# catid/siamese

Hardware: AMD Instinct MI355X
Metric: device-resident GB/s encode+decode, 1400B pkts @20% loss; % HBM peak (higher is better)
Workload: dtype u8

## Files before the change

### siamese_amd/csrc/engine.cpp

```cpp
#include "engine.h"

#include <pthread.h>
#include "backend.h"
#include "codedef.h"
#include "pool.h"

#include <algorithm>
#include <chrono>
#include <cmath>
#include <cstdio>
#include <cstddef>
#include <cstdlib>
#include <cstring>

#ifndef SGPU_EXEC_LPT
#define SGPU_EXEC_LPT 1
#endif
#ifndef SGPU_EXEC_GROUPS
#define SGPU_EXEC_GROUPS 256
#endif

namespace sgpu {

void EngineStats::add(const EngineStats& o)
// ... 28 lines not shown
namespace {

uint64_t now_ns()
{
    return (uint64_t)std::chrono::duration_cast<std::chrono::nanoseconds>(
               std::chrono::steady_clock::now().time_since_epoch())
        .count();
}

inline size_t align16(size_t v) { return (v + 15) & ~(size_t)15; }

}


namespace {
std::mutex g_bodyMu;
std::vector<ProgramBody*> g_bodies;
}

ProgramBody* ProgramBody::get()
{
    {
        std::lock_guard<std::mutex> g(g_bodyMu);
        if (!g_bodies.empty()) {
            ProgramBody* b = g_bodies.back();
            g_bodies.pop_back();
            return b;
        }
    }
    return new ProgramBody;
}

void ProgramBody::put(ProgramBody* b)
{
    b->clear();
    std::lock_guard<std::mutex> g(g_bodyMu);
    if (g_bodies.size() < (1u << 15))
        g_bodies.push_back(b);
    else
        delete b;
}

void ProgramBody::clear()
{
    for (size_t k = 0; k < nsegs; ++k)
        segs[k].clear();
    nsegs = 0;
    resultWords = 0;
    nsolves = 0;
    nges = 0;
    callbacks.clear();
    keep.clear();
    rb.open = false;
    rb.win.clear();
    rb.updates.clear();
    rb.rows.clear();
    copies.clear();
    lcb.clear();
    ndeliver = 0;
    nframe = 0;
    frameLit.clear();
    frameLitRefs.clear();
    nrelay = 0;
    npackjob = npack = 0;
    nconcatjob = nconcat = 0;
    gateOpen = false;
}

void ProgramBody::new_segment()
{
    rows_close();
    if (nsegs == segs.size())
        segs.emplace_back();
    segs[nsegs++].clear();
}

void ProgramBody::rows_open(uint32_t base, bool keepWindow)
{
    rows_close();
    if (nsegs == 0)
        new_segment();
    rb.open = true;
    rb.haveSums = false;
    rb.sumsVersion = 0;
    rb.readMask = 0;
    rb.cutMax = 0;
    rb.versioned = false;
    if (!keepWindow) {
        rb.base = base;
        rb.win.clear();
    }
    rb.updates.clear();
    for (int& u : rb.updateOf)
        u = -1;
    rb.rows.clear();
    rb.maxExtent = 0;
}

namespace {
inline bool overlaps(uint64_t a, uint64_t an, uint64_t b, uint64_t bn) { return a < b + bn && b < a + an; }
inline uint64_t lane_span(uint32_t n) { return ((uint64_t)n + 15) & ~(uint64_t)15; }
}

void ProgramBody::lc_seal()
{
    if (lcb.items.empty())
        return;
    Segment& s = segs[nsegs - 1];
    if (lcb.items.size() == 1) {
        const LcItem& it = lcb.items[0];
        GfOp op;
        std::memset(&op, 0, sizeof(op));
        op.dst = it.dst;
        op.n = it.n;
        op.valid = it.valid;
        op.kind = OP_LINCOMB;
        op.mix = it.mixLit & 0xff;
        op.termBegin = (uint32_t)s.terms.size();
        op.termCount = it.termCount;
        s.ops.push_back(op);
        s.terms.insert(s.terms.end(), lcb.terms.begin(), lcb.terms.end());
        const uint32_t litLen = (it.mixLit >> 8) & 0xff;
        if (litLen) {
            GfOp lo;
            std::memset(&lo, 0, sizeof(lo));
            lo.dst = it.dst;
            lo.n = it.litOffset;
            lo.valid = litLen;
            lo.kind = OP_LITERAL;
            std::memcpy(lo.lit, it.lit, litLen);
            s.ops.push_back(lo);
        }
        lcb.clear();
        return;
    }
    const uint32_t itemWords = (uint32_t)lcb.items.size() * kLcWords;
    for (LcItem& it : lcb.items)
        it.termStart += itemWords;
    GfOp op;
    std::memset(&op, 0, sizeof(op));
    op.kind = OP_LINCOMBS;
    op.n = (uint32_t)lcb.items.size();
    op.termBegin = (uint32_t)(s.rowsData.size() / 16);
    op.termCount = itemWords + (uint32_t)lcb.terms.size();
    s.ops.push_back(op);
    const size_t at = s.rowsData.size();
    s.rowsData.resize(at + (size_t)op.termCount * 16);
    std::memcpy(s.rowsData.data() + at, lcb.items.data(), lcb.items.size() * sizeof(LcItem));
    std::memcpy(s.rowsData.data() + at + lcb.items.size() * sizeof(LcItem), lcb.terms.data(),
                lcb.terms.size() * sizeof(GfTerm));
    s.rowsWords += op.termCount;
    lcb.clear();
}

namespace {

using Span = ProgramBody::LcBuild::Span;

bool span_hits(const std::vector<Span>& v, uint64_t lo, uint64_t hi)
{
    const auto it = std::upper_bound(v.begin(), v.end(), lo,
                                     [](uint64_t x, const Span& sp) { return x < sp.hi; });
    return it != v.end() && it->lo < hi;
}

void span_add(std::vector<Span>& v, uint64_t lo, uint64_t hi)
{
    if (lo >= hi)
        return;
    auto first = std::lower_bound(v.begin(), v.end(), lo,
                                  [](const Span& sp, uint64_t x) { return sp.hi < x; });
    auto last = first;
    while (last != v.end() && last->lo <= hi) {
        lo = std::min(lo, last->lo);
        hi = std::max(hi, last->hi);
        ++last;
    }
    if (first == last) {
        v.insert(first, Span{lo, hi});
    } else {
        *first = Span{lo, hi};
        v.erase(first + 1, last);
    }
}

uint64_t lc_write_span(const LcItem& it)
{
    const uint32_t litEnd = it.litOffset + ((it.mixLit >> 8) & 0xff);
    return std::max<uint64_t>(lane_span(it.n), litEnd);
}

}

void ProgramBody::lc_absorb()
{
    static const bool enabled = [] {
        const char* v = std::getenv("SIAMESE_AMD_LC_BATCH");
        return !v || std::atoi(v) != 0;
    }();
    if (!enabled)
        return;
    Segment& s = segs[nsegs - 1];
    const GfOp op = s.ops.back();
// ... 6 lines not shown
    }
    bool indep = lcb.items.size() < kLcMaxItems;
    const uint64_t w = lane_span(op.n);
    if (indep && !lcb.items.empty()) {
        if (span_hits(lcb.writes, op.dst, op.dst + w) || span_hits(lcb.reads, op.dst, op.dst + w))
            indep = false;
        for (uint32_t k = 0; indep && k < op.termCount; ++k)
            if (span_hits(lcb.writes, t[k].src, t[k].src + lane_span(t[k].len)))
                indep = false;
        const LcItem& it = lcb.items.back();
        const uint64_t iw = lc_write_span(it);
        if (indep && overlaps(op.dst, w, it.dst, iw))
            indep = false;
        for (uint32_t k = 0; indep && k < op.termCount; ++k)
            if (overlaps(t[k].src, lane_span(t[k].len), it.dst, iw))
                indep = false;
        const GfTerm* u = lcb.terms.data() + it.termStart;
        for (uint32_t k = 0; indep && k < it.termCount; ++k)
            if (overlaps(u[k].src, lane_span(u[k].len), op.dst, w))
                indep = false;
    }
    lcScratch.assign(t, t + op.termCount);
    s.terms.resize(op.termBegin);
    s.ops.pop_back();
    if (!indep) {
        lc_seal();
    } else if (!lcb.items.empty()) {
        const LcItem& it = lcb.items.back();
        span_add(lcb.writes, it.dst, it.dst + lc_write_span(it));
        const GfTerm* u = lcb.terms.data() + it.termStart;
        for (uint32_t k = 0; k < it.termCount; ++k)
            span_add(lcb.reads, u[k].src, u[k].src + lane_span(u[k].len));
    }
    LcItem it;
    std::memset(&it, 0, sizeof(it));
    it.dst = op.dst;
    it.n = op.n;
    it.valid = op.valid;
    it.termStart = (uint32_t)lcb.terms.size();
    it.termCount = op.termCount;
    it.mixLit = op.mix & 0xff;
    lcb.items.push_back(it);
    lcb.terms.insert(lcb.terms.end(), lcScratch.begin(), lcScratch.end());
}

bool ProgramBody::lc_literal_fits(uint64_t at, uint32_t len) const
{
    return !span_hits(lcb.writes, at, at + len) && !span_hits(lcb.reads, at, at + len);
}

void ProgramBody::rows_close()
{
    lc_seal();
    if (!copies.empty()) {
        Segment& g = segs[nsegs - 1];
        GfOp op;
        std::memset(&op, 0, sizeof(op));
        op.kind = OP_COPIES;
        op.n = (uint32_t)copies.size();
        op.termBegin = (uint32_t)(g.rowsData.size() / 16);
        op.termCount = (uint32_t)copies.size() * kCopyWords;
        g.ops.push_back(op);
        const size_t at = g.rowsData.size();
        g.rowsData.resize(at + copies.size() * sizeof(CopyItem));
        std::memcpy(g.rowsData.data() + at, copies.data(), copies.size() * sizeof(CopyItem));
        g.rowsWords += op.termCount;
        copies.clear();
    }
    RowsBuild& b = rb;
    if (!b.open)
        return;
    b.open = false;
    if (b.rows.empty() && b.updates.empty())
        return;
    if (!b.haveSums)
        std::memset(b.sums, 0, sizeof(b.sums));
    Segment& s = segs[nsegs - 1];
    const size_t winKept = b.win.size();
    for (RowItem& r : b.rows) {
        if (r.ldpcN < kLdpcSplitMin)
            continue;
        const uint32_t entry = (uint32_t)b.win.size();
        const uint32_t pairs = (r.ldpcN + kPairRate - 1) / kPairRate;
        s.wide.push_back(Segment::Wide{(uint32_t)s.ops.size(), entry, r.n, r.row, r.ldpcN, r.ldpcOff});
        s.wideItems += ((r.n + kLdpcTileBytes - 1) / kLdpcTileBytes) *
                       ((pairs + ldpc_pairs_per_item(r.n) - 1) / ldpc_pairs_per_item(r.n));
        s.wideBytes += 2 * (uint64_t)((r.n + kLdpcTileBytes - 1) / kLdpcTileBytes * kLdpcTileBytes);
        WinEntry z;
        std::memset(&z, 0, sizeof(z));
        b.win.push_back(z);
        b.win.push_back(z);
        r.ldpcN = 0;
        r.ldpcOff = entry;
        r.mask0 |= kRowWide;
    }
    const uint32_t E = (uint32_t)b.win.size();
    const uint32_t U = (uint32_t)b.updates.size();
    const uint32_t R = (uint32_t)b.rows.size();
    const uint32_t words = kRowSums + E + U * kUpdateWords + R * kRowWords;
    uint32_t stageLo = E;
    for (const SumUpdate& u : b.updates)
        if (u.to > u.from)
            stageLo = std::min(stageLo, u.from);
    for (const RowItem& r : b.rows)
        if (r.ldpcN || (r.mask0 & kRowWide))
            stageLo = std::min(stageLo, r.ldpcOff);
    GfOp op;
    std::memset(&op, 0, sizeof(op));
    op.dst = stageLo | (uint64_t)(b.versioned ? std::min<uint32_t>(R, kVersionRows) : 0u) << 32;
    op.kind = OP_ROWS;
    op.n = R;
    op.valid = E;
    op.mix = U;
    op.termBegin = (uint32_t)(s.rowsData.size() / 16);
    op.termCount = words;
    s.ops.push_back(op);
    const size_t at = s.rowsData.size();
    s.rowsData.resize(at + (size_t)words * 16);
    uint8_t* w = s.rowsData.data() + at;
    std::memcpy(w, b.sums, sizeof(b.sums));
    w += sizeof(b.sums);
    std::memcpy(w, b.win.data(), (size_t)E * sizeof(WinEntry));
    w += (size_t)E * sizeof(WinEntry);
    std::memcpy(w, b.updates.data(), (size_t)U * sizeof(SumUpdate));
    w += (size_t)U * sizeof(SumUpdate);
    std::memcpy(w, b.rows.data(), (size_t)R * sizeof(RowItem));
    b.win.resize(winKept);
    s.rowsWords += words;
    if (b.maxExtent > s.maxExtent)
        s.maxExtent = b.maxExtent;
}


Program::~Program()
{
    if (!shard_) {
        if (b_)
            ProgramBody::put(b_);
        return;
    }
    Program* orphan = new Program(eng_, group_ | 2);
    orphan->shard_ = shard_;
    orphan->b_ = b_;
    b_ = nullptr;
    std::lock_guard<std::mutex> g(shard_->mu);
    auto it = std::find(shard_->dirty.begin(), shard_->dirty.end(), this);
    if (it != shard_->dirty.end())
        *it = orphan;
}

void Program::attach()
{
    if (!b_)
        b_ = ProgramBody::get();
    b_->group = group_ & 1;
    Shard& s = eng_->shard();
    shard_ = &s;
    std::lock_guard<std::mutex> g(s.mu);
    s.dirty.push_back(this);
}

void Program::lc_begin(uint64_t dst, uint32_t n, uint32_t valid, uint8_t mix)
{
    touch();
    if (b_->rb.open || !b_->copies.empty()) {
        b_->lc_seal();
        b_->rows_close();
    }
    if (b_->nsegs == 0)
        b_->new_segment();
    ProgramBody::Segment& s = b_->segs[b_->nsegs - 1];
    GfOp op;
    op.dst = dst;
    op.n = n;
    op.valid = valid < n ? valid : n;
    op.kind = OP_LINCOMB;
    op.mix = mix;
    op.termBegin = (uint32_t)s.terms.size();
    op.termCount = 0;
    s.ops.push_back(op);
}

void Program::lc_end()
{
    ProgramBody::Segment& s = b_->segs[b_->nsegs - 1];
    GfOp& op = s.ops.back();
    if (op.termCount == 0 && op.valid >= op.n) {
        s.ops.pop_back();
        return;
    }
    if (op.n > s.maxExtent)
        s.maxExtent = op.n;
    b_->lc_absorb();
}

void Program::add_mem(uint64_t dst, uint64_t src, uint32_t n)
{
    if (n == 0)
        return;
    lc_begin(dst, n, n);
    lc_term(src, n, 1);
    lc_end();
}

void Program::muladd_mem(uint64_t dst, uint8_t y, uint64_t src, uint32_t n)
{
    if (n == 0 || y == 0)
        return;
    lc_begin(dst, n, n);
    lc_term(src, n, y);
    lc_end();
}

void Program::mul_mem(uint64_t dst, uint64_t src, uint8_t y, uint32_t n)
{
    if (n == 0)
        return;
    lc_begin(dst, n, 0);
// ... 50 lines not shown

void Program::ingest_device(const DevBuf& dst, uint64_t src, uint32_t bytes, const uint8_t* hdr,
                            uint32_t hdrLen)
{
    ingest_run(dst.addr(), 0, src, 0, 1, bytes, hdr, hdrLen);
}

void Program::ingest_run(uint64_t dst, uint32_t dstStride, uint64_t src, uint32_t srcStride, uint32_t count,
                         uint32_t bytes, const uint8_t* hdr, uint32_t hdrLen)
{
    IngestDesc d;
    std::memset(&d, 0, sizeof(d));
    d.dst = dst;
    d.src = src;
    d.bytes = bytes;
    d.hdrLen = hdrLen;
    d.count = count;
    d.srcStride = count > 1 ? srcStride : 0;
    d.dstStride = count > 1 ? dstStride : 0;
    std::memcpy(d.hdr, hdr, hdrLen < 8 ? hdrLen : 8);
    eng_->add_ingest(d, -1);
}

uint32_t Program::solve(const std::vector<SolveRow>& rows, const uint8_t* coef, uint32_t maxBytes)
{
    SolveRow* r = nullptr;
    uint8_t* c = nullptr;
    solve_reserve((unsigned)rows.size(), &r, &c);
    std::memcpy(r, rows.data(), rows.size() * sizeof(SolveRow));
    std::memcpy(c, coef, rows.size() * rows.size());
    return solve_commit(maxBytes);
}

void Program::solve_reserve(unsigned m, SolveRow** rows, uint8_t** coef)
{
    touch();
    if (b_->nsegs == 0)
        b_->new_segment();
    if (b_->nsolves == b_->solves.size())
        b_->solves.emplace_back();
    ProgramBody::PendingSolve& ps = b_->solves[b_->nsolves];
    ps.rows.resize(m);
    ps.coef.resize((size_t)m * m);
    *rows = ps.rows.data();
    *coef = ps.coef.data();
}

uint32_t Program::solve_commit(uint32_t maxBytes, uint32_t gateWord)
{
    ProgramBody::PendingSolve& ps = b_->solves[b_->nsolves++];
    const size_t m = ps.rows.size();
    DevBuf head = eng_->alloc((uint32_t)m * 16u);
    if (head) {
        if (b_->copies.empty()) {
            b_->rows_close();
            if (b_->nsegs == 0)
                b_->new_segment();
        }
        std::vector<CopyItem>& cp = b_->copies;
        size_t at = cp.size();
        cp.resize(at + m);
        uint32_t ext = 0;
        for (size_t i = 0; i < m; ++i) {
            const uint32_t len = std::min<uint32_t>(16u, ps.rows[i].initBytes);
            if (len == 0)
                continue;
            CopyItem& c = cp[at++];
            std::memset(&c, 0, sizeof(c));
            c.dst = head.addr() + i * 16;
            c.src = ps.rows[i].buf;
            c.len = len;
            ext = std::max(ext, len);
        }
        cp.resize(at);
        ProgramBody::Segment& g = b_->segs[b_->nsegs - 1];
        if (ext > g.maxExtent)
            g.maxExtent = ext;
        b_->rows_close();
    }
    std::memset(&ps.desc, 0, sizeof(ps.desc));
    ps.desc.head = head.addr();
    eng_->release(head);
    ps.desc.m = (uint32_t)m;
    ps.desc.maxBytes = maxBytes;
    ps.desc.gate = gateWord;
    if (gateWord && b_->nges) {
        ProgramBody::PendingGe& g = b_->ges[b_->nges - 1];
        g.solve = (uint32_t)(b_->nsolves - 1);
    }
    ps.desc.result = b_->resultWords;
    b_->resultWords += ps.desc.m + 2;
    const uint32_t r = ps.desc.result;
    b_->new_segment();
    return r;
}

void Program::gate_begin(uint32_t word)
{
    touch();
    b_->rows_close();
    if (b_->nsegs == 0)
        b_->new_segment();
    b_->gateOpen = true;
    b_->gateSeg = b_->nsegs - 1;
    b_->gateOp = (uint32_t)b_->segs[b_->nsegs - 1].ops.size();
    b_->gateWord = word;
}

uint32_t Program::gate_end()
{
    if (!b_ || !b_->gateOpen)
        return 0;
    b_->rows_close();
    b_->gateOpen = false;
    ProgramBody::Segment& s = b_->segs[b_->gateSeg];
    uint32_t wide = 0;
    if (b_->gateSeg + 1 == b_->nsegs && s.ops.size() > b_->gateOp) {
        s.gates.push_back(ProgramBody::Segment::Gate{b_->gateOp, (uint32_t)s.ops.size(), b_->gateWord});
        for (const ProgramBody::Segment::Wide& x : s.wide)
            wide += x.op >= b_->gateOp;
    }
    return wide;
}

uint8_t* Program::ge_job(unsigned rows, unsigned cols, unsigned pickLen, uint32_t* resultWord, bool chained)
{
    touch();
    if (b_->nges == b_->ges.size())
        b_->ges.emplace_back();
    ProgramBody::PendingGe& g = b_->ges[b_->nges++];
    g.rows = (uint16_t)rows;
    g.cols = (uint16_t)cols;
    g.pickLen = pickLen;
    g.result = b_->resultWords;
    g.chained = chained;
    g.solve = ~0u;
    b_->resultWords += ge_result_words(rows, cols, chained);
    g.in.resize(ge_input_bytes(rows, cols, pickLen));
    *resultWord = g.result;
    return g.in.data();
}

void Program::on_complete(Completion fn)
{
    touch();
    b_->callbacks.push_back(std::move(fn));
}

void Program::on_complete(std::shared_ptr<void> keep, Completion fn)
{
    touch();
    b_->keep.push_back(std::move(keep));
    b_->callbacks.push_back(std::move(fn));
}


WinEntry* Program::rows_window(uint32_t lo, uint32_t hi, uint32_t* from)
{
    touch();
    ProgramBody::RowsBuild& b = b_->rb;
    if (!b.open || lo < b.base)
        rows_open(lo, false);
    const uint32_t end = b.base + (uint32_t)b.win.size();
    if (hi <= end) {
        *from = hi;
        return nullptr;
    }
    *from = end;
    b.win.resize(hi - b.base);
    return b.win.data() + (end - b.base);
}

void Program::rows_update(unsigned k, uint64_t dst, uint32_t n, uint32_t valid, unsigned s,
                          uint32_t fromElement, uint32_t toElement)
{
    ProgramBody::RowsBuild& b = b_->rb;
    if (b.readMask >> k & 1) {
        const WinEntry& seen = b.sums[k];
        if (seen.src != dst || valid < seen.len || toElement - fromElement > kVersionMaxSpan ||
            b.rows.size() >= kVersionRows)
            rows_open(b.base, true);
        else
            b.versioned = true;
    }
    const uint32_t from = fromElement - b.base, to = toElement - b.base;
    int& ui = b.updateOf[k];
    if (ui >= 0) {
        SumUpdate& u = b.updates[ui];
        const uint64_t d = ((uint64_t)u.dstHi << 32) | u.dstLo;
        if (d == dst && (u.to == from || from == to)) {
            if (from != to)
                u.to = to;
            if (n > u.n)
                u.n = n;
            if (n > b.maxExtent)
                b.maxExtent = n;
            return;
        }
        rows_open(b.base, true);
    }
    SumUpdate u;
    std::memset(&u, 0, sizeof(u));
    u.dstLo = (uint32_t)dst;
    u.dstHi = (uint32_t)(dst >> 32);
    u.n = n;
    u.valid = valid < n ? valid : n;
    u.s = s;
    u.from = from;
    u.to = to < from ? from : to;
    u.sum = k;
    b.updateOf[k] = (int)b.updates.size();
    b.updates.push_back(u);
    if (n > b.maxExtent)
        b.maxExtent = n;
}

uint64_t Program::next_table_version()
{
    static std::atomic<uint64_t> next{1};
    return next.fetch_add(1, std::memory_order_relaxed);
}

void Program::rows_row(const WinEntry* sums, uint64_t dst, uint32_t n, uint32_t valid, uint8_t mix,
                       uint32_t mask0, uint32_t mask1, unsigned row, uint32_t ldpcN,
                       uint32_t ldpcFirst, uint32_t cutoff, const uint8_t* lit, uint32_t litLen,
                       uint64_t sumsVersion)
{
    ProgramBody::RowsBuild& b = b_->rb;
    const bool unchanged = sumsVersion != 0 && b.haveSums && b.sumsVersion == sumsVersion;
    bool same = true;
    if (b.haveSums && !unchanged)
        for (uint32_t r = b.readMask; r; r &= r - 1) {
            const unsigned k = (unsigned)__builtin_ctz(r);
            if (std::memcmp(&b.sums[k], &sums[k], sizeof(WinEntry)) != 0) {
                same = false;
                break;
            }
        }
    if (!same || cutoff < b.cutMax || (b.versioned && b.rows.size() >= kVersionRows))
        rows_open(b.base, true);
    b.cutMax = std::max(b.cutMax, cutoff);
    if (!(unchanged && b.haveSums))
        std::memcpy(b.sums, sums, sizeof(b.sums));
    b.haveSums = true;
    b.sumsVersion = sumsVersion;
    RowItem r;
    std::memset(&r, 0, sizeof(r));
    r.dst = dst;
    r.n = n;
    r.valid = valid < n ? valid : n;
    r.mask0 = mask0 | (litLen << 24);
    r.mask1 = mask1 | ((uint32_t)mix << 24);
    r.row = row;
    r.ldpcN = ldpcN;
    r.ldpcOff = ldpcFirst - b.base;
    r.cutoff = cutoff - b.base;
    if (litLen)
        std::memcpy(r.lit, lit, litLen);
    b.rows.push_back(r);
    b.readMask |= mask0 | mask1;
    if (n + litLen > b.maxExtent)
        b.maxExtent = n + litLen;
}

void Program::copy(uint64_t dst, uint64_t src, uint32_t len)
{
    if (len == 0)
        return;
    touch();
    if (b_->copies.empty()) {
        b_->rows_close();
        if (b_->nsegs == 0)
            b_->new_segment();
    }
    CopyItem c;
    std::memset(&c, 0, sizeof(c));
    c.dst = dst;
    c.src = src;
    c.len = len;
    b_->copies.push_back(c);
    ProgramBody::Segment& g = b_->segs[b_->nsegs - 1];
    if (len > g.maxExtent)
        g.maxExtent = len;
}

void Program::deliver(uint64_t src, uint32_t cap, uint64_t dst, uint64_t lenOut, uint64_t stride)
{
    touch();
    DeliverItem it;
    it.src = src;
    it.dst = dst;
    it.lenOut = lenOut;
    it.cap = cap;
    it.stride16 = (uint32_t)(stride >> 4);
    if (b_->ndeliver == b_->delivers.size())
        b_->delivers.emplace_back();
    b_->delivers[b_->ndeliver++] = it;
}

void Program::frame(uint64_t src, uint32_t bytes, const uint8_t* hdr, uint32_t hdrLen, uint64_t dst,
                    uint64_t lenOut, uint64_t stride, uint32_t lenBase)
{
    touch();
    FrameItem it;
    it.src = src;
    it.dst = dst;
    it.lenOut = lenOut;
    it.bytes = bytes;
    it.stride16 = (uint32_t)(stride >> 4);
    std::memset(it.hdr, 0, sizeof(it.hdr));
    std::memcpy(it.hdr, hdr, hdrLen);
    it.hdrLen = (uint8_t)hdrLen;
    it.lenBase = lenBase;
    if (b_->nframe == b_->frames.size())
        b_->frames.emplace_back();
    b_->frames[b_->nframe++] = it;
}

void Program::frame_literal(const uint8_t* data, uint32_t bytes, const uint8_t* hdr, uint32_t hdrLen, uint64_t dst,
                            uint64_t lenOut, uint64_t stride)
{
    touch();
    const size_t at = b_->frameLit.size();
    b_->frameLit.resize(align16(at + bytes), 0);
    std::memcpy(b_->frameLit.data() + at, data, bytes);
    b_->frameLitRefs.push_back(ProgramBody::FrameLitRef{b_->nframe, (uint32_t)at});
    frame(1 , bytes, hdr, hdrLen, dst, lenOut, stride);
}

void Program::relay(uint64_t src, uint32_t cap, uint32_t flow, uint32_t packetNum, uint64_t dst, uint64_t lenOut,
                    uint64_t stride)
{
    touch();
    RelayItem it;
// ... 615 lines not shown
constexpr size_t kAcctBytes = 32;

constexpr size_t kParallelWords = 1u << 16;
#ifndef SGPU_SEAL_CHUNK
#define SGPU_SEAL_CHUNK 32
#endif
#ifndef SGPU_SEG_CHUNK
#define SGPU_SEG_CHUNK 16
#endif
#ifndef SGPU_INGEST_CHUNK
#define SGPU_INGEST_CHUNK 8192
#endif
#ifndef SGPU_SOLVE_CHUNK
#define SGPU_SOLVE_CHUNK 64
#endif

std::atomic<bool> g_measureUnique{false};

struct Range
{
    uint64_t addr;
    uint32_t len;
};

uint64_t distinct_bytes(std::vector<Range>& v)
{
    std::sort(v.begin(), v.end(), [](const Range& a, const Range& b) { return a.addr < b.addr; });
    uint64_t total = 0;
    for (size_t i = 0; i < v.size();) {
        uint32_t len = v[i].len;
        size_t j = i + 1;
        for (; j < v.size() && v[j].addr == v[i].addr; ++j)
            len = std::max(len, v[j].len);
        total += len;
        i = j;
    }
    return total;
}

uint64_t segment_unique_bytes(const ProgramBody::Segment& s, std::vector<Range>& rd, std::vector<Range>& wr)
{
    rd.clear();
    wr.clear();
    uint64_t words = 0;
    auto R = [&](uint64_t a, uint32_t n) {
        if (a && n)
            rd.push_back(Range{a, n});
    };
    auto W = [&](uint64_t a, uint32_t n, uint32_t valid) {
        if (a && n)
            wr.push_back(Range{a, n});
        R(a, std::min(valid, n));
    };
    for (const GfOp& op : s.ops) {
        words += op_words(op);
        const uint8_t* blk = s.rowsData.data() + (size_t)op.termBegin * 16;
        switch (op.kind) {
        case OP_LINCOMB:
            W(op.dst, op.n, op.valid);
            for (uint32_t t = 0; t < op.termCount; ++t)
                R(s.terms[op.termBegin + t].src, s.terms[op.termBegin + t].len);
            break;
        case OP_LITERAL:
            W(op.dst + op.n, op.valid, 0);
            break;
        case OP_ROWS: {
            const WinEntry* sums = reinterpret_cast<const WinEntry*>(blk);
            const WinEntry* win = sums + kRowSums;
            const SumUpdate* up = reinterpret_cast<const SumUpdate*>(win + op.valid);
            const RowItem* rows = reinterpret_cast<const RowItem*>(up + op.mix);
            for (unsigned k = 0; k < kRowSums; ++k)
                R(sums[k].src, sums[k].len);
            for (uint32_t e = (uint32_t)op.dst; e < op.valid; ++e)
                R(win[e].src, win[e].len);
            for (uint32_t u = 0; u < op.mix; ++u)
                W((uint64_t)up[u].dstHi << 32 | up[u].dstLo, up[u].n, up[u].valid);
            for (uint32_t r = 0; r < op.n; ++r)
                W(rows[r].dst, rows[r].n + row_lit_len(rows[r].mask0), rows[r].valid);
            break;
        }
        case OP_COPIES: {
            const CopyItem* c = reinterpret_cast<const CopyItem*>(blk);
            for (uint32_t i = 0; i < op.n; ++i) {
                W(c[i].dst, c[i].len, 0);
                R(c[i].src, c[i].len);
            }
            break;
        }
        case OP_LINCOMBS: {
            const LcItem* it = reinterpret_cast<const LcItem*>(blk);
            for (uint32_t i = 0; i < op.n; ++i) {
                W(it[i].dst, std::max(it[i].n, it[i].litOffset + ((it[i].mixLit >> 8) & 0xff)), it[i].valid);
                const GfTerm* t = reinterpret_cast<const GfTerm*>(blk + (size_t)it[i].termStart * 16);
                for (uint32_t k = 0; k < it[i].termCount; ++k)
                    R(t[k].src, t[k].len);
            }
            break;
        }
        default:
            break;
        }
    }
    return words * 16 + distinct_bytes(rd) + distinct_bytes(wr);
}

}

void Engine::set_measure_unique(bool on) { g_measureUnique.store(on, std::memory_order_relaxed); }
bool Engine::measure_unique() { return g_measureUnique.load(std::memory_order_relaxed); }

void Engine::start_threads()
{
    stop_ = false;
    launcher_ = std::thread([this] {
        pthread_setname_np(pthread_self(), "sgpu-launch");
        launcher_loop();
    });
    completer_ = std::thread([this] {
        pthread_setname_np(pthread_self(), "sgpu-complete");
        completer_loop();
    });
}

// ... 281 lines not shown
                launching_ = false;
                continue;
            }
        }
        if (!b->assembled && !failed()) {
            claim_set(*b);
            assemble_batch(*b, asm_pool());
            tl("assembled", b->ticket);
        }
        tl("launch begin", b->ticket);
        if (!failed())
            launch_batch(*b);
        tl("launch end", b->ticket);
        {
            std::lock_guard<std::mutex> g(qMu_);
            toComplete_.push_back(b);
            launching_ = false;
        }
        completeCv_.notify_one();
    }
}

void Engine::claim_set(Batch& b)
{
    std::unique_lock<std::mutex> lk(qMu_);
    setCv_.wait(lk, [&] { return stop_ || sets_[b.set].busyTicket == 0; });
    sets_[b.set].busyTicket = b.ticket;
}

WorkerPool& Engine::asm_pool()
{
    if (!asmPool_) {
        const char* v = std::getenv("SIAMESE_AMD_ASM_THREADS");
        const int n = v ? std::atoi(v) : 4;
        asmPool_.reset(new WorkerPool((unsigned)std::max(1, std::min(64, n)), 0, "sgpu-assemble"));
    }
    return *asmPool_;
}

void Engine::assemble_batch(Batch& bt, WorkerPool& wp)
{
    bt.assembled = true;
    const uint64_t t0 = now_ns();
    XferSet& xs = sets_[bt.set];
    EngineStats& st = bt.st;
    size_t totalBodies = bt.bodies[0].size() + bt.bodies[1].size();
    size_t approxWords = 0;
    for (const Shard::Queues& q : bt.queues)
        approxWords += q.ingest.size() * 2;
    for (int g = 0; g < 2; ++g)
        for (ProgramBody* p : bt.bodies[g])
            for (size_t k = 0; k < p->nsegs; ++k)
                approxWords += p->segs[k].ops.size() * 2 + p->segs[k].terms.size() +
                               p->segs[k].rowsWords + p->rb.win.size() + p->rb.rows.size() * 3;
    const bool parallel = approxWords >= kParallelWords;
    auto run = [&](size_t n, const std::function<void(size_t)>& fn) {
        if (parallel)
            wp.run(n, fn);
        else
            for (size_t i = 0; i < n; ++i)
                fn(i);
    };

    constexpr size_t kSealChunk = SGPU_SEAL_CHUNK;
    run((totalBodies + kSealChunk - 1) / kSealChunk, [&](size_t c) {
        for (size_t i = c * kSealChunk; i < std::min(totalBodies, c * kSealChunk + kSealChunk); ++i) {
            const size_t n0 = bt.bodies[0].size();
            (i < n0 ? bt.bodies[0][i] : bt.bodies[1][i - n0])->rows_close();
        }
    });

    uint32_t resultWords = 0;
    for (int g = 0; g < 2; ++g)
        for (ProgramBody* p : bt.bodies[g]) {
            bt.resultBase[g].push_back(resultWords);
            resultWords += p->resultWords;
        }
    bt.resultWords = resultWords;

    std::vector<SegRef> segs;
    std::vector<Phase>& phases = bt.phases;
    std::vector<SolveDesc> sdescs;
    struct SolveRef
    {
        const ProgramBody::PendingSolve* ps;
        size_t rowBase, coefBase;
    };
    std::vector<SolveRef> srefs;
    size_t nSolveRows = 0, nCoef = 0;
    std::vector<SolveItem> sitems;
    size_t nOps = 0, nTerms = 0, nWords = 0, nItems = 0, nWide = 0;
    uint64_t wideBytes = 0, tBytes = 0;
    uint64_t rowsShape[kRowsShapeStats] = {0, 0, 0, 0, 0};
    const uint32_t stageCap = be_exec_stage_cap();
    for (int g = 0; g < 2; ++g) {
        size_t maxSegs = 0;
        for (ProgramBody* p : bt.bodies[g])
            maxSegs = std::max(maxSegs, p->nsegs);
        for (size_t k = 0; k < maxSegs; ++k) {
            Phase ex{Phase::EXEC, nItems, 0, 0, 0, kNoRows};
            const size_t segBegin = segs.size();
            for (size_t pi = 0; pi < bt.bodies[g].size(); ++pi) {
                const ProgramBody* p = bt.bodies[g][pi];
                if (k >= p->nsegs)
                    continue;
                const ProgramBody::Segment& s = p->segs[k];
                if (s.ops.empty())
// ... 266 lines not shown
        bt.wideBase = xs.wideUsed;
        xs.wideUsed += need;
    }
    if (tBytes) {
        ensure_solve(xs, tBytes);
        const uint64_t tBase = (uint64_t)(uintptr_t)xs.solveDev;
        for (SolveDesc& d : sdescs)
            if (d.tinv) {
                d.tinv = tBase + (d.tinv - 1);
                d.xout = tBase + (d.xout - 1);
            }
    }

    uint8_t* up = xs.upHost;
    const uint64_t stageDev = (uint64_t)(uintptr_t)(bt.upBase + oStage);
    constexpr size_t kSegChunk = SGPU_SEG_CHUNK;
    constexpr size_t kSolveChunk = SGPU_SOLVE_CHUNK;
    struct Task
    {
        int kind;
        size_t a, b;
    };
    std::vector<Task> tasks;
    for (size_t i = 0; i < segs.size(); i += kSegChunk)
        tasks.push_back(Task{0, i, std::min(segs.size(), i + kSegChunk)});
    for (size_t i = 0; i < grefs.size(); i += kSolveChunk)
        tasks.push_back(Task{3, i, std::min(grefs.size(), i + kSolveChunk)});
    for (size_t i = 0; i < srefs.size(); i += kSolveChunk)
        tasks.push_back(Task{2, i, std::min(srefs.size(), i + kSolveChunk)});
    for (size_t qi = 0; qi < bt.queues.size(); ++qi)
        for (size_t c = 0; c < std::max<size_t>(1, bt.queues[qi].ingest.size()); c += kIngestChunk)
            tasks.push_back(Task{1, qi, c});
    const bool measureUnique = measure_unique();
    std::atomic<uint64_t> uniqueBytes{0};
    run(tasks.size(), [&](size_t ti) {
        const Task& t = tasks[ti];
        if (t.kind == 0) {
            if (measureUnique) {
                std::vector<Range> rd, wr;
                uint64_t u = 0;
                for (size_t si = t.a; si < t.b; ++si)
                    u += segment_unique_bytes(*segs[si].seg, rd, wr);
                uniqueBytes.fetch_add(u, std::memory_order_relaxed);
            }
            for (size_t si = t.a; si < t.b; ++si) {
                const SegRef& r = segs[si];
                const ProgramBody::Segment& s = *r.seg;
                uint8_t* w = up + bt.oStream + (size_t)r.wordBase * 16;
                size_t wi = 0;
                LdpcItem* wItem = (LdpcItem*)(up + bt.oWide) + r.wideBase;
                uint32_t* wGate = bt.wideGated ? (uint32_t*)(up + bt.oWideGate) + r.wideBase : nullptr;
                uint64_t wOff = bt.wideBase + r.wideOff;
                size_t gi = 0;
                for (uint32_t oi = 0; oi < (uint32_t)s.ops.size(); ++oi) {
                    const GfOp& op = s.ops[oi];
                    std::memcpy(w, &op, sizeof(GfOp));
                    uint32_t opGate = 0;
                    if (op.kind != OP_LITERAL) {
                        while (gi < s.gates.size() && s.gates[gi].opEnd <= oi)
                            ++gi;
                        const bool gated = gi < s.gates.size() && s.gates[gi].opBegin <= oi;
                        opGate = gated ? 1u + s.gates[gi].word + r.resultBase : 0u;
                        reinterpret_cast<GfOp*>(w)->termBegin = opGate;
                    }
                    w += sizeof(GfOp);
                    if (op.kind == OP_ROWS || op.kind == OP_COPIES || op.kind == OP_LINCOMBS) {
                        const size_t bytes = (size_t)op.termCount * 16;
                        std::memcpy(w, s.rowsData.data() + (size_t)op.termBegin * 16, bytes);
                        const uint64_t winDev = (uint64_t)(uintptr_t)(bt.upBase + (w - up)) + kRowSums * 16;
                        for (; wi < s.wide.size() && s.wide[wi].op == oi; ++wi) {
                            const ProgramBody::Segment::Wide& x = s.wide[wi];
                            const uint32_t span = (x.n + kLdpcTileBytes - 1) / kLdpcTileBytes * kLdpcTileBytes;
                            const uint64_t dst = (uint64_t)(uintptr_t)xs.wideDev + wOff;
                            wOff += 2 * (uint64_t)span;
                            WinEntry* e = reinterpret_cast<WinEntry*>(w + (size_t)(kRowSums + x.entry) * 16);
                            e[0].src = dst;
                            e[0].len = x.n;
                            e[1].src = dst + span;
                            e[1].len = x.n;
                            const uint32_t pairs = (x.N + kPairRate - 1) / kPairRate;
                            const uint32_t ppi = ldpc_pairs_per_item(x.n);
                            for (uint32_t t = 0; t < x.n; t += kLdpcTileBytes)
                                for (uint32_t p0 = 0; p0 < pairs; p0 += ppi) {
                                    LdpcItem& it = *wItem++;
                                    it.win = winDev;
                                    it.dst = dst;
                                    it.span = span;
                                    it.n = x.n;
                                    it.row = x.row;
                                    it.N = x.N;
                                    it.off = x.off;
                                    it.tileBase = t;
                                    it.pair0 = p0;
                                    it.pair1 = std::min(pairs, p0 + ppi);
                                    if (wGate)
                                        *wGate++ = opGate;
                                }
                        }
                        w += bytes;
                    } else if (op.kind == OP_LINCOMB && op.termCount) {
                        const size_t bytes = (size_t)op.termCount * sizeof(GfTerm);
                        std::memcpy(w, s.terms.data() + op.termBegin, bytes);
                        w += bytes;
                    }
                }
                ExecItem* items = (ExecItem*)(up + bt.oItems) + r.itemBase;
                const uint32_t nOpsSeg = (uint32_t)s.ops.size();
                const uint32_t tiles = (s.maxExtent + kExecTileBytes - 1) / kExecTileBytes;
                uint32_t n = 0;
                for (uint32_t t = 0; t < tiles; t += r.tilesPerItem)
                    items[n++] = ExecItem{r.wordBase, r.words, nOpsSeg,
                                          exec_tiles(t, std::min(r.tilesPerItem, tiles - t))};
            }
        } else if (t.kind == 3) {
            for (size_t i = t.a; i < t.b; ++i) {
                uint8_t* in = up + bt.oGeIn + grefs[i].inOff;
                if (grefs[i].cancelled) {
                    std::memset(in, 0, ge_input_bytes(1, 1, 0));
                    GeRow* r = reinterpret_cast<GeRow*>(in);
                    r->kind = GE_PARITY;
                    r->colCount = 1;
// ... 621 lines not shown
```

### siamese_amd/csrc/engine.h

```cpp
#pragma once

#include "ops.h"

#include <atomic>
#include <condition_variable>
#include <cstdint>
#include <cstdio>
#include <cstdlib>
#include <deque>
#include <functional>
#include <memory>
#include <mutex>
#include <pthread.h>
#include <shared_mutex>
#include <thread>
#include <vector>

namespace sgpu {

class InstanceLock
{
public:
    InstanceLock() = default;
    InstanceLock(const InstanceLock&) = delete;
// ... 94 lines not shown
            std::this_thread::yield();
    }
    void wait_writer()
    {
        for (unsigned spin = 0; spin < 512; ++spin) {
            if (writer_.load(std::memory_order_seq_cst) == 0)
                return;
            __builtin_ia32_pause();
        }
        std::unique_lock<std::mutex> lk(cvMu_);
        waiters_.fetch_add(1, std::memory_order_seq_cst);
        cv_.wait(lk, [&] { return writer_.load(std::memory_order_seq_cst) == 0; });
        waiters_.fetch_sub(1, std::memory_order_relaxed);
    }

    Slot slots_[kSlots];
    alignas(64) std::atomic<int> writer_{0};
    std::atomic<int> waiters_{0};
    std::mutex wmu_;
    std::mutex cvMu_;
    std::condition_variable cv_;
};

class WorkerPool;

struct DevBuf
{
    uint8_t* ptr = nullptr;
    uint32_t cap = 0;
    explicit operator bool() const { return ptr != nullptr; }
    uint64_t addr() const { return (uint64_t)(uintptr_t)ptr; }
};

uint32_t round_cap(uint32_t bytes);

struct Slab
{
    DevBuf buf;
    uint32_t stride = 0;
    uint64_t used = 0;
};

constexpr uint32_t kSlabMinSlot = 1408;
inline uint32_t slab_stride(uint32_t need)
{
    const uint32_t stride = round_cap(need > kSlabMinSlot ? need : kSlabMinSlot);
    return (uint64_t)stride * 64 > 0xffffffffu ? 0 : stride;
}

class Engine;
struct Shard;
struct Batch;

using Completion = std::function<void(const uint32_t* results)>;

struct ProgramBody
{
    struct Segment
    {
        std::vector<GfOp> ops;
        std::vector<GfTerm> terms;
        std::vector<uint8_t> rowsData;
        uint32_t rowsWords = 0;
        uint32_t maxExtent = 0;
        struct Wide
        {
            uint32_t op;
            uint32_t entry;
            uint32_t n, row, N, off;
        };
        std::vector<Wide> wide;
        uint32_t wideItems = 0;
        uint64_t wideBytes = 0;
        struct Gate
        {
            uint32_t opBegin, opEnd, word;
        };
        std::vector<Gate> gates;
        void clear()
        {
            ops.clear();
            terms.clear();
            rowsData.clear();
            rowsWords = 0;
            maxExtent = 0;
            wide.clear();
            wideItems = 0;
            wideBytes = 0;
            gates.clear();
        }
    };
    struct RowsBuild
    {
        bool open = false;
        bool haveSums = false;
        uint64_t sumsVersion = 0;
        WinEntry sums[kRowSums];
        uint32_t readMask = 0;
        uint32_t cutMax = 0;
        bool versioned = false;
        uint32_t base = 0;
        std::vector<WinEntry> win;
        std::vector<SumUpdate> updates;
        int updateOf[kRowSums];
        std::vector<RowItem> rows;
        uint32_t maxExtent = 0;
    };
    struct PendingSolve
    {
        SolveDesc desc;
        std::vector<SolveRow> rows;
        std::vector<uint8_t> coef;
        mutable uint32_t asmRow = 0, asmCoef = 0;
    };
    struct PendingGe
    {
        uint16_t rows = 0, cols = 0;
        uint32_t pickLen = 0;
        uint32_t result = 0;
        bool chained = false;
        uint32_t solve = ~0u;
        std::vector<uint8_t> in;
    };

    int group = 0;
    uint32_t resultWords = 0;
    size_t nsegs = 0;
    std::vector<Segment> segs;
    std::vector<PendingSolve> solves;
    size_t nsolves = 0;
    std::vector<PendingGe> ges;
    uint32_t nges = 0;
    uint32_t ndeliver = 0;
    uint32_t nframe = 0;
    uint32_t nrelay = 0;
    std::vector<Completion> callbacks;
    std::vector<std::shared_ptr<void>> keep;
    RowsBuild rb;
    bool gateOpen = false;
    size_t gateSeg = 0;
    uint32_t gateOp = 0, gateWord = 0;
    std::vector<CopyItem> copies;
    struct LcBuild
    {
        std::vector<LcItem> items;
        std::vector<GfTerm> terms;
        struct Span
        {
            uint64_t lo, hi;
        };
        std::vector<Span> writes, reads;
        void clear()
        {
            items.clear();
            terms.clear();
            writes.clear();
            reads.clear();
        }
    } lcb;
    std::vector<GfTerm> lcScratch;
    std::vector<DeliverItem> delivers;
    std::vector<FrameItem> frames;
    struct FrameLitRef
    {
        uint32_t item;
        uint32_t offset;
    };
    std::vector<uint8_t> frameLit;
    std::vector<FrameLitRef> frameLitRefs;
    std::vector<RelayItem> relays;
    std::vector<PackJob> packJobs;
    std::vector<PackItem> packs;
    uint32_t npackjob = 0, npack = 0;
    std::vector<ConcatJob> concatJobs;
    std::vector<ConcatItem> concats;
    uint32_t nconcatjob = 0, nconcat = 0;
    void lc_seal();
    void lc_absorb();
    bool lc_literal_fits(uint64_t at, uint32_t len) const;

    bool empty() const
    {
        return nges == 0 && ndeliver == 0 && nframe == 0 && nrelay == 0 && npackjob == 0 &&
               nconcatjob == 0 &&
               (nsegs == 0 ||
                (nsegs == 1 && segs[0].ops.empty() && copies.empty() && lcb.items.empty() && !rb.open));
    }
    void new_segment();
    void rows_open(uint32_t base, bool keepWindow);
    void rows_close();
    void clear();

    static ProgramBody* get();
    static void put(ProgramBody* b);
};

class Program
{
public:
    Program(Engine* e, int group) : eng_(e), group_(group) {}
    ~Program();
    Program(const Program&) = delete;
    Program& operator=(const Program&) = delete;

    int group() const { return group_; }

    void lc_begin(uint64_t dst, uint32_t n, uint32_t valid, uint8_t mix = 0);
    void lc_term(uint64_t src, uint32_t len, uint8_t coeff, uint8_t acc = 0)
    {
        ProgramBody::Segment& s = b_->segs[b_->nsegs - 1];
        GfOp& op = s.ops.back();
        if (len > op.n)
            len = op.n;
        if (len == 0 || coeff == 0)
            return;
        GfTerm t;
        t.src = src;
        t.len = len;
        t.coeff = coeff;
        t.acc = acc;
        t.pad = 0;
        s.terms.push_back(t);
        ++op.termCount;
    }
    void lc_end();

    void add_mem(uint64_t dst, uint64_t src, uint32_t n);
    void muladd_mem(uint64_t dst, uint8_t y, uint64_t src, uint32_t n);
    void mul_mem(uint64_t dst, uint64_t src, uint8_t y, uint32_t n);
    void zero(uint64_t dst, uint32_t n);

    void literal(uint64_t dst, uint32_t offset, const uint8_t* bytes, uint32_t len);

    void ingest_host(const DevBuf& dst, const void* data, uint32_t bytes, const uint8_t* hdr,
                     uint32_t hdrLen);
    void ingest_device(const DevBuf& dst, uint64_t src, uint32_t bytes, const uint8_t* hdr,
                       uint32_t hdrLen);
    void ingest_run(uint64_t dst, uint32_t dstStride, uint64_t src, uint32_t srcStride, uint32_t count,
                    uint32_t bytes, const uint8_t* hdr, uint32_t hdrLen);
// ... 336 lines not shown
```

Baseline: 4170.

## Build row op blocks in place in segment buffers instead of staging vectors

Replaces the per-rows-build staging vectors (window, updates, rows, copies) with in-place writes into a realloc-backed POD buffer owned by each segment, with updates and row items stored in separate per-segment arrays. This removes the extra copy at rows_close and the value-initialization cost of std::vector resize on the host program-building path. Upload then stitches the header, updates and rows together. The risk is more complex bookkeeping (block offsets, memmove of the kept window on reopen, pointer invalidation after grow).

```diff
diff --git a/siamese_amd/csrc/engine.cpp b/siamese_amd/csrc/engine.cpp
--- a/siamese_amd/csrc/engine.cpp
+++ b/siamese_amd/csrc/engine.cpp
@@ -104,10 +104,8 @@
     callbacks.clear();
     keep.clear();
     rb.open = false;
-    rb.win.clear();
-    rb.updates.clear();
-    rb.rows.clear();
-    copies.clear();
+    rb.winCount = 0;
+    ncopies = 0;
     lcb.clear();
     ndeliver = 0;
     nframe = 0;
@@ -140,12 +138,19 @@
     rb.versioned = false;
     if (!keepWindow) {
         rb.base = base;
-        rb.win.clear();
-    }
-    rb.updates.clear();
+        rb.winCount = 0;
+    }
+    Segment& s = segs[nsegs - 1];
+    const size_t keptAt = rb.blockAt + sizeof(WinEntry) * kRowSums;
+    rb.blockAt = s.rowsData.size();
+    s.rowsData.grow(sizeof(WinEntry) * ((size_t)kRowSums + rb.winCount));
+    if (rb.winCount)
+        std::memmove(s.rowsData.data() + rb.blockAt + sizeof(WinEntry) * kRowSums, s.rowsData.data() + keptAt,
+                     sizeof(WinEntry) * (size_t)rb.winCount);
+    rb.updBegin = s.rowUpdates.size();
+    rb.rowBegin = s.rowItems.size();
     for (int& u : rb.updateOf)
         u = -1;
-    rb.rows.clear();
     rb.maxExtent = 0;
 }
 
@@ -196,11 +201,9 @@
     op.termBegin = (uint32_t)(s.rowsData.size() / 16);
     op.termCount = itemWords + (uint32_t)lcb.terms.size();
     s.ops.push_back(op);
-    const size_t at = s.rowsData.size();
-    s.rowsData.resize(at + (size_t)op.termCount * 16);
-    std::memcpy(s.rowsData.data() + at, lcb.items.data(), lcb.items.size() * sizeof(LcItem));
-    std::memcpy(s.rowsData.data() + at + lcb.items.size() * sizeof(LcItem), lcb.terms.data(),
-                lcb.terms.size() * sizeof(GfTerm));
+    uint8_t* blk = s.rowsData.grow((size_t)op.termCount * 16);
+    std::memcpy(blk, lcb.items.data(), lcb.items.size() * sizeof(LcItem));
+    std::memcpy(blk + lcb.items.size() * sizeof(LcItem), lcb.terms.data(), lcb.terms.size() * sizeof(GfTerm));
     s.rowsWords += op.termCount;
     lcb.clear();
 }
@@ -313,59 +316,60 @@
 void ProgramBody::rows_close()
 {
     lc_seal();
-    if (!copies.empty()) {
+    if (ncopies) {
         Segment& g = segs[nsegs - 1];
         GfOp op;
         std::memset(&op, 0, sizeof(op));
         op.kind = OP_COPIES;
-        op.n = (uint32_t)copies.size();
-        op.termBegin = (uint32_t)(g.rowsData.size() / 16);
-        op.termCount = (uint32_t)copies.size() * kCopyWords;
+        op.n = ncopies;
+        op.termBegin = (uint32_t)(copyAt / 16);
+        op.termCount = ncopies * kCopyWords;
         g.ops.push_back(op);
-        const size_t at = g.rowsData.size();
-        g.rowsData.resize(at + copies.size() * sizeof(CopyItem));
-        std::memcpy(g.rowsData.data() + at, copies.data(), copies.size() * sizeof(CopyItem));
         g.rowsWords += op.termCount;
-        copies.clear();
+        ncopies = 0;
     }
     RowsBuild& b = rb;
     if (!b.open)
         return;
     b.open = false;
-    if (b.rows.empty() && b.updates.empty())
+    Segment& s = segs[nsegs - 1];
+    const size_t R0 = s.rowItems.size() - b.rowBegin;
+    if (R0 == 0 && s.rowUpdates.size() == b.updBegin) {
+        s.rowsData.n = b.blockAt;
         return;
+    }
     if (!b.haveSums)
-        std::memset(b.sums, 0, sizeof(b.sums));
-    Segment& s = segs[nsegs - 1];
-    const size_t winKept = b.win.size();
-    for (RowItem& r : b.rows) {
+        std::memset(s.rowsData.data() + b.blockAt, 0, sizeof(WinEntry) * kRowSums);
+    const uint32_t winKept = b.winCount;
+    for (size_t ri = 0; ri < R0; ++ri) {
+        RowItem& r = s.rowItems.data()[b.rowBegin + ri];
         if (r.ldpcN < kLdpcSplitMin)
             continue;
-        const uint32_t entry = (uint32_t)b.win.size();
+        const uint32_t entry = b.winCount;
         const uint32_t pairs = (r.ldpcN + kPairRate - 1) / kPairRate;
         s.wide.push_back(Segment::Wide{(uint32_t)s.ops.size(), entry, r.n, r.row, r.ldpcN, r.ldpcOff});
         s.wideItems += ((r.n + kLdpcTileBytes - 1) / kLdpcTileBytes) *
                        ((pairs + ldpc_pairs_per_item(r.n) - 1) / ldpc_pairs_per_item(r.n));
         s.wideBytes += 2 * (uint64_t)((r.n + kLdpcTileBytes - 1) / kLdpcTileBytes * kLdpcTileBytes);
-        WinEntry z;
-        std::memset(&z, 0, sizeof(z));
-        b.win.push_back(z);
-        b.win.push_back(z);
+        std::memset(s.rowsData.grow(2 * sizeof(WinEntry)), 0, 2 * sizeof(WinEntry));
+        b.winCount += 2;
         r.ldpcN = 0;
         r.ldpcOff = entry;
         r.mask0 |= kRowWide;
     }
-    const uint32_t E = (uint32_t)b.win.size();
-    const uint32_t U = (uint32_t)b.updates.size();
-    const uint32_t R = (uint32_t)b.rows.size();
+    const uint32_t E = b.winCount;
+    const uint32_t U = (uint32_t)(s.rowUpdates.size() - b.updBegin);
+    const uint32_t R = (uint32_t)R0;
+    const SumUpdate* updates = s.rowUpdates.data() + b.updBegin;
+    const RowItem* rows = s.rowItems.data() + b.rowBegin;
     const uint32_t words = kRowSums + E + U * kUpdateWords + R * kRowWords;
     uint32_t stageLo = E;
-    for (const SumUpdate& u : b.updates)
-        if (u.to > u.from)
-            stageLo = std::min(stageLo, u.from);
-    for (const RowItem& r : b.rows)
-        if (r.ldpcN || (r.mask0 & kRowWide))
-            stageLo = std::min(stageLo, r.ldpcOff);
+    for (uint32_t i = 0; i < U; ++i)
+        if (updates[i].to > updates[i].from)
+            stageLo = std::min(stageLo, updates[i].from);
+    for (uint32_t i = 0; i < R; ++i)
+        if (rows[i].ldpcN || (rows[i].mask0 & kRowWide))
+            stageLo = std::min(stageLo, rows[i].ldpcOff);
     GfOp op;
     std::memset(&op, 0, sizeof(op));
     op.dst = stageLo | (uint64_t)(b.versioned ? std::min<uint32_t>(R, kVersionRows) : 0u) << 32;
@@ -373,20 +377,10 @@
     op.n = R;
     op.valid = E;
     op.mix = U;
-    op.termBegin = (uint32_t)(s.rowsData.size() / 16);
+    op.termBegin = (uint32_t)(b.blockAt / 16);
     op.termCount = words;
     s.ops.push_back(op);
-    const size_t at = s.rowsData.size();
-    s.rowsData.resize(at + (size_t)words * 16);
-    uint8_t* w = s.rowsData.data() + at;
-    std::memcpy(w, b.sums, sizeof(b.sums));
-    w += sizeof(b.sums);
-    std::memcpy(w, b.win.data(), (size_t)E * sizeof(WinEntry));
-    w += (size_t)E * sizeof(WinEntry);
-    std::memcpy(w, b.updates.data(), (size_t)U * sizeof(SumUpdate));
-    w += (size_t)U * sizeof(SumUpdate);
-    std::memcpy(w, b.rows.data(), (size_t)R * sizeof(RowItem));
-    b.win.resize(winKept);
+    b.winCount = winKept;
     s.rowsWords += words;
     if (b.maxExtent > s.maxExtent)
         s.maxExtent = b.maxExtent;
@@ -424,7 +418,7 @@
 void Program::lc_begin(uint64_t dst, uint32_t n, uint32_t valid, uint8_t mix)
 {
     touch();
-    if (b_->rb.open || !b_->copies.empty()) {
+    if (b_->rb.open || b_->ncopies) {
         b_->lc_seal();
         b_->rows_close();
     }
@@ -581,14 +575,15 @@
     const size_t m = ps.rows.size();
     DevBuf head = eng_->alloc((uint32_t)m * 16u);
     if (head) {
-        if (b_->copies.empty()) {
+        if (b_->ncopies == 0) {
             b_->rows_close();
             if (b_->nsegs == 0)
                 b_->new_segment();
-        }
-        std::vector<CopyItem>& cp = b_->copies;
-        size_t at = cp.size();
-        cp.resize(at + m);
+            b_->copyAt = b_->segs[b_->nsegs - 1].rowsData.size();
+        }
+        ProgramBody::Segment& g = b_->segs[b_->nsegs - 1];
+        CopyItem* cp = reinterpret_cast<CopyItem*>(g.rowsData.grow(m * sizeof(CopyItem)));
+        size_t at = 0;
         uint32_t ext = 0;
         for (size_t i = 0; i < m; ++i) {
             const uint32_t len = std::min<uint32_t>(16u, ps.rows[i].initBytes);
@@ -601,8 +596,8 @@
             c.len = len;
             ext = std::max(ext, len);
         }
-        cp.resize(at);
-        ProgramBody::Segment& g = b_->segs[b_->nsegs - 1];
+        g.rowsData.n -= (m - at) * sizeof(CopyItem);
+        b_->ncopies += (uint32_t)at;
         if (ext > g.maxExtent)
             g.maxExtent = ext;
         b_->rows_close();
@@ -690,14 +685,14 @@
     ProgramBody::RowsBuild& b = b_->rb;
     if (!b.open || lo < b.base)
         rows_open(lo, false);
-    const uint32_t end = b.base + (uint32_t)b.win.size();
+    const uint32_t end = b.base + b.winCount;
     if (hi <= end) {
         *from = hi;
         return nullptr;
     }
     *from = end;
-    b.win.resize(hi - b.base);
-    return b.win.data() + (end - b.base);
+    b.winCount = hi - b.base;
+    return reinterpret_cast<WinEntry*>(b_->segs[b_->nsegs - 1].rowsData.grow(sizeof(WinEntry) * (size_t)(hi - end)));
 }
 
 void Program::rows_update(unsigned k, uint64_t dst, uint32_t n, uint32_t valid, unsigned s,
@@ -705,9 +700,10 @@
 {
     ProgramBody::RowsBuild& b = b_->rb;
     if (b.readMask >> k & 1) {
-        const WinEntry& seen = b.sums[k];
+        ProgramBody::Segment& g = b_->segs[b_->nsegs - 1];
+        const WinEntry& seen = reinterpret_cast<const WinEntry*>(g.rowsData.data() + b.blockAt)[k];
         if (seen.src != dst || valid < seen.len || toElement - fromElement > kVersionMaxSpan ||
-            b.rows.size() >= kVersionRows)
+            g.rowItems.size() - b.rowBegin >= kVersionRows)
             rows_open(b.base, true);
         else
             b.versioned = true;
@@ -715,7 +711,7 @@
     const uint32_t from = fromElement - b.base, to = toElement - b.base;
     int& ui = b.updateOf[k];
     if (ui >= 0) {
-        SumUpdate& u = b.updates[ui];
+        SumUpdate& u = b_->segs[b_->nsegs - 1].rowUpdates.data()[b.updBegin + ui];
         const uint64_t d = ((uint64_t)u.dstHi << 32) | u.dstLo;
         if (d == dst && (u.to == from || from == to)) {
             if (from != to)
@@ -728,7 +724,9 @@
         }
         rows_open(b.base, true);
     }
-    SumUpdate u;
+    ProgramBody::Segment& seg = b_->segs[b_->nsegs - 1];
+    b.updateOf[k] = (int)(seg.rowUpdates.size() - b.updBegin);
+    SumUpdate& u = *seg.rowUpdates.grow(1);
     std::memset(&u, 0, sizeof(u));
     u.dstLo = (uint32_t)dst;
     u.dstHi = (uint32_t)(dst >> 32);
@@ -738,8 +736,6 @@
     u.from = from;
     u.to = to < from ? from : to;
     u.sum = k;
-    b.updateOf[k] = (int)b.updates.size();
-    b.updates.push_back(u);
     if (n > b.maxExtent)
         b.maxExtent = n;
 }
@@ -758,22 +754,28 @@
     ProgramBody::RowsBuild& b = b_->rb;
     const bool unchanged = sumsVersion != 0 && b.haveSums && b.sumsVersion == sumsVersion;
     bool same = true;
-    if (b.haveSums && !unchanged)
+    if (b.haveSums && !unchanged) {
+        const ProgramBody::Segment& g = b_->segs[b_->nsegs - 1];
+        const WinEntry* have = reinterpret_cast<const WinEntry*>(g.rowsData.data() + b.blockAt);
         for (uint32_t r = b.readMask; r; r &= r - 1) {
             const unsigned k = (unsigned)__builtin_ctz(r);
-            if (std::memcmp(&b.sums[k], &sums[k], sizeof(WinEntry)) != 0) {
+            if (std::memcmp(&have[k], &sums[k], sizeof(WinEntry)) != 0) {
                 same = false;
                 break;
             }
         }
-    if (!same || cutoff < b.cutMax || (b.versioned && b.rows.size() >= kVersionRows))
+    }
+    ProgramBody::Segment* seg = &b_->segs[b_->nsegs - 1];
+    if (!same || cutoff < b.cutMax || (b.versioned && seg->rowItems.size() - b.rowBegin >= kVersionRows)) {
         rows_open(b.base, true);
+        seg = &b_->segs[b_->nsegs - 1];
+    }
     b.cutMax = std::max(b.cutMax, cutoff);
     if (!(unchanged && b.haveSums))
-        std::memcpy(b.sums, sums, sizeof(b.sums));
+        std::memcpy(seg->rowsData.data() + b.blockAt, sums, sizeof(WinEntry) * kRowSums);
     b.haveSums = true;
     b.sumsVersion = sumsVersion;
-    RowItem r;
+    RowItem& r = *seg->rowItems.grow(1);
     std::memset(&r, 0, sizeof(r));
     r.dst = dst;
     r.n = n;
@@ -786,7 +788,6 @@
     r.cutoff = cutoff - b.base;
     if (litLen)
         std::memcpy(r.lit, lit, litLen);
-    b.rows.push_back(r);
     b.readMask |= mask0 | mask1;
     if (n + litLen > b.maxExtent)
         b.maxExtent = n + litLen;
@@ -797,18 +798,19 @@
     if (len == 0)
         return;
     touch();
-    if (b_->copies.empty()) {
+    if (b_->ncopies == 0) {
         b_->rows_close();
         if (b_->nsegs == 0)
             b_->new_segment();
-    }
-    CopyItem c;
+        b_->copyAt = b_->segs[b_->nsegs - 1].rowsData.size();
+    }
+    ProgramBody::Segment& g = b_->segs[b_->nsegs - 1];
+    CopyItem& c = *reinterpret_cast<CopyItem*>(g.rowsData.grow(sizeof(CopyItem)));
     std::memset(&c, 0, sizeof(c));
     c.dst = dst;
     c.src = src;
     c.len = len;
-    b_->copies.push_back(c);
-    ProgramBody::Segment& g = b_->segs[b_->nsegs - 1];
+    ++b_->ncopies;
     if (len > g.maxExtent)
         g.maxExtent = len;
 }
@@ -1530,6 +1532,7 @@
             wr.push_back(Range{a, n});
         R(a, std::min(valid, n));
     };
+    size_t updAt = 0, rowAt = 0;
     for (const GfOp& op : s.ops) {
         words += op_words(op);
         const uint8_t* blk = s.rowsData.data() + (size_t)op.termBegin * 16;
@@ -1545,8 +1548,10 @@
         case OP_ROWS: {
             const WinEntry* sums = reinterpret_cast<const WinEntry*>(blk);
             const WinEntry* win = sums + kRowSums;
-            const SumUpdate* up = reinterpret_cast<const SumUpdate*>(win + op.valid);
-            const RowItem* rows = reinterpret_cast<const RowItem*>(up + op.mix);
+            const SumUpdate* up = s.rowUpdates.data() + updAt;
+            const RowItem* rows = s.rowItems.data() + rowAt;
+            updAt += op.mix;
+            rowAt += op.n;
             for (unsigned k = 0; k < kRowSums; ++k)
                 R(sums[k].src, sums[k].len);
             for (uint32_t e = (uint32_t)op.dst; e < op.valid; ++e)
@@ -1934,7 +1939,8 @@
         for (ProgramBody* p : bt.bodies[g])
             for (size_t k = 0; k < p->nsegs; ++k)
                 approxWords += p->segs[k].ops.size() * 2 + p->segs[k].terms.size() +
-                               p->segs[k].rowsWords + p->rb.win.size() + p->rb.rows.size() * 3;
+                               p->segs[k].rowsWords + p->rb.winCount +
+                               (p->rb.open && k + 1 == p->nsegs ? (p->segs[k].rowItems.size() - p->rb.rowBegin) * 3 : 0);
     const bool parallel = approxWords >= kParallelWords;
     auto run = [&](size_t n, const std::function<void(size_t)>& fn) {
         if (parallel)
@@ -2307,6 +2313,7 @@
                 uint32_t* wGate = bt.wideGated ? (uint32_t*)(up + bt.oWideGate) + r.wideBase : nullptr;
                 uint64_t wOff = bt.wideBase + r.wideOff;
                 size_t gi = 0;
+                size_t updAt = 0, rowAt = 0;
                 for (uint32_t oi = 0; oi < (uint32_t)s.ops.size(); ++oi) {
                     const GfOp& op = s.ops[oi];
                     std::memcpy(w, &op, sizeof(GfOp));
@@ -2321,7 +2328,18 @@
                     w += sizeof(GfOp);
                     if (op.kind == OP_ROWS || op.kind == OP_COPIES || op.kind == OP_LINCOMBS) {
                         const size_t bytes = (size_t)op.termCount * 16;
-                        std::memcpy(w, s.rowsData.data() + (size_t)op.termBegin * 16, bytes);
+                        const uint8_t* blk = s.rowsData.data() + (size_t)op.termBegin * 16;
+                        if (op.kind == OP_ROWS) {
+                            const size_t head = ((size_t)kRowSums + op.valid) * sizeof(WinEntry);
+                            const size_t ub = (size_t)op.mix * sizeof(SumUpdate), rbytes = (size_t)op.n * sizeof(RowItem);
+                            std::memcpy(w, blk, head);
+                            std::memcpy(w + head, s.rowUpdates.data() + updAt, ub);
+                            std::memcpy(w + head + ub, s.rowItems.data() + rowAt, rbytes);
+                            updAt += op.mix;
+                            rowAt += op.n;
+                        } else {
+                            std::memcpy(w, blk, bytes);
+                        }
                         const uint64_t winDev = (uint64_t)(uintptr_t)(bt.upBase + (w - up)) + kRowSums * 16;
                         for (; wi < s.wide.size() && s.wide[wi].op == oi; ++wi) {
                             const ProgramBody::Segment::Wide& x = s.wide[wi];
diff --git a/siamese_amd/csrc/engine.h b/siamese_amd/csrc/engine.h
--- a/siamese_amd/csrc/engine.h
+++ b/siamese_amd/csrc/engine.h
@@ -170,6 +170,47 @@
 struct Shard;
 struct Batch;
 
+template <class T>
+struct PodVec
+{
+    T* p = nullptr;
+    size_t n = 0, cap = 0;
+    PodVec() = default;
+    PodVec(PodVec&& o) noexcept : p(o.p), n(o.n), cap(o.cap) { o.p = nullptr, o.n = o.cap = 0; }
+    PodVec& operator=(PodVec&& o) noexcept
+    {
+        if (this != &o) {
+            std::free(p);
+            p = o.p, n = o.n, cap = o.cap;
+            o.p = nullptr, o.n = o.cap = 0;
+        }
+        return *this;
+    }
+    PodVec(const PodVec&) = delete;
+    PodVec& operator=(const PodVec&) = delete;
+    ~PodVec() { std::free(p); }
+    T* grow(size_t k)
+    {
+        if (n + k > cap) {
+            size_t c = cap ? cap * 2 : 4096 / sizeof(T);
+            while (c < n + k)
+                c *= 2;
+            T* q = static_cast<T*>(std::realloc(p, c * sizeof(T)));
+            if (!q)
+                std::abort();
+            p = q, cap = c;
+        }
+        T* r = p + n;
+        n += k;
+        return r;
+    }
+    void clear() { n = 0; }
+    bool empty() const { return n == 0; }
+    size_t size() const { return n; }
+    T* data() { return p; }
+    const T* data() const { return p; }
+};
+
 using Completion = std::function<void(const uint32_t* results)>;
 
 struct ProgramBody
@@ -178,7 +219,9 @@
     {
         std::vector<GfOp> ops;
         std::vector<GfTerm> terms;
-        std::vector<uint8_t> rowsData;
+        PodVec<uint8_t> rowsData;
+        PodVec<SumUpdate> rowUpdates;
+        PodVec<RowItem> rowItems;
         uint32_t rowsWords = 0;
         uint32_t maxExtent = 0;
         struct Wide
@@ -200,6 +243,8 @@
             ops.clear();
             terms.clear();
             rowsData.clear();
+            rowUpdates.clear();
+            rowItems.clear();
             rowsWords = 0;
             maxExtent = 0;
             wide.clear();
@@ -213,15 +258,15 @@
         bool open = false;
         bool haveSums = false;
         uint64_t sumsVersion = 0;
-        WinEntry sums[kRowSums];
         uint32_t readMask = 0;
         uint32_t cutMax = 0;
         bool versioned = false;
         uint32_t base = 0;
-        std::vector<WinEntry> win;
-        std::vector<SumUpdate> updates;
+        size_t blockAt = 0;
+        uint32_t winCount = 0;
+        size_t updBegin = 0;
+        size_t rowBegin = 0;
         int updateOf[kRowSums];
-        std::vector<RowItem> rows;
         uint32_t maxExtent = 0;
     };
     struct PendingSolve
@@ -258,7 +303,8 @@
     bool gateOpen = false;
     size_t gateSeg = 0;
     uint32_t gateOp = 0, gateWord = 0;
-    std::vector<CopyItem> copies;
+    uint32_t ncopies = 0;
+    size_t copyAt = 0;
     struct LcBuild
     {
         std::vector<LcItem> items;
@@ -302,7 +348,7 @@
         return nges == 0 && ndeliver == 0 && nframe == 0 && nrelay == 0 && npackjob == 0 &&
                nconcatjob == 0 &&
                (nsegs == 0 ||
-                (nsegs == 1 && segs[0].ops.empty() && copies.empty() && lcb.items.empty() && !rb.open));
+                (nsegs == 1 && segs[0].ops.empty() && ncopies == 0 && lcb.items.empty() && !rb.open));
     }
     void new_segment();
     void rows_open(uint32_t base, bool keepWindow);
```

Result: faster. 4298 (median of 6 runs) (+3.1%).
